# jbikker/tinybvh

Hardware: NVIDIA H100
Metric: Mrays/s (primary+shadow) (higher is better)
Workload: dtype f32

## Files before the change

### tinybvh_b200/csrc/api.cu

```cuda
#include "common.cuh"
#include <stdarg.h>
#include <stdlib.h>
#include <string.h>
#include <vector>
#include <thread>
#include <atomic>
#include <mutex>
#include <condition_variable>
#include <memory>
#include <functional>
#include <new>

static thread_local char g_err[512] = "";
unsigned long long g_tbvh_launches = 0;

void tbvh_set_error( const char* fmt, ... )
{
	va_list ap;
	va_start( ap, fmt );
	vsnprintf( g_err, sizeof( g_err ), fmt, ap );
	va_end( ap );
}

#define ARG_CHECK( c, msg ) do { if (!(c)) { tbvh_set_error( "%s: %s", __func__, msg ); return TBVH_E_ARG; } } while (0)
// ... 670 lines not shown
	ARG_CHECK( instance && blas, "NULL argument" );
	if (!(blas->info.layouts & (1u << TBVH_LAYOUT_BVH))) { tbvh_set_error( "tbvh_instance_update: the BLAS holds no tree" ); return TBVH_E_STATE; }
	return tbvh_instance_update_box( instance, blas->info.aabb_min, blas->info.aabb_max );
}

int tbvh_build_tlas( tbvh_bvh t, const void* instances, uint32_t inst_stride, uint32_t inst_count, const tbvh_bvh* blasses, uint32_t blas_count, float c_trav, float c_int )
{
	ARG_CHECK( t && instances && blasses && inst_count > 0 && blas_count > 0 && inst_stride >= 160, "bad TLAS arguments" );
	CUDA_TRY( cudaSetDevice( t->ctx->device ) );
	free_layouts( t );
	std::vector<float4> boxes( (size_t)inst_count * 2 );
	std::vector<TlasInst> inst( inst_count );
	std::vector<BlasRef> refs( blas_count );
	uint32_t blas_layouts = (1u << TBVH_LAYOUT_BVH) | (1u << TBVH_LAYOUT_CWBVH);
	for (uint32_t k = 0; k < blas_count; k++)
	{
		const tbvh_bvh b = blasses[k];
		ARG_CHECK( b && b != t && b->ctx == t->ctx, "TLAS: a BLAS handle is NULL or lives in another context" );
		const bool has_bvh = (b->info.layouts & (1u << TBVH_LAYOUT_BVH)) && b->d_trav && b->d_leaf_tris, has_cw = b->d_cw_trav && b->d_cw_tris;
		if (b->d_inst || (!has_bvh && !has_cw))
		{ tbvh_set_error( "TLAS: BLAS %u holds no triangle tree (IntersectTLAS walks LAYOUT_BVH BLASses, tiny_bvh.h:3341; traverse_tlas.cl CWBVH ones)", k ); return TBVH_E_STATE; }
		if (has_bvh && b->info.max_depth + 1 > TBVH_STACK) { tbvh_set_error( "TLAS: BLAS %u has depth %u, the two-level kernel walks a BLAS with a %d-entry stack", k, b->info.max_depth, TBVH_STACK ); return TBVH_E_LIMIT; }
		if (has_cw && b->cw_depth + 1 > 128) { tbvh_set_error( "TLAS: the wide tree of BLAS %u has depth %u (128 pending node groups per ray, tiny_bvh.h:7048)", k, b->cw_depth ); return TBVH_E_LIMIT; }
		refs[k].trav = has_bvh ? b->d_trav : 0, refs[k].tris = has_bvh ? b->d_leaf_tris : 0, refs[k].root_ref = b->root_ref, refs[k].root_count = b->root_count, refs[k].pad0 = refs[k].pad1 = 0;
		refs[k].cw_nodes = has_cw ? b->d_cw_trav : 0, refs[k].cw_tris = has_cw ? b->d_cw_tris : 0;
		blas_layouts &= (has_bvh ? 1u << TBVH_LAYOUT_BVH : 0u) | (has_cw ? 1u << TBVH_LAYOUT_CWBVH : 0u);
	}
	for (uint32_t i = 0; i < inst_count; i++)
	{
		const char* r = (const char*)instances + (size_t)i * inst_stride;
		memcpy( inst[i].inv, r + 64, 64 );
		memcpy( &inst[i].blasIdx, r + 140, 4 ), memcpy( &inst[i].mask, r + 156, 4 );
		inst[i].pad0 = inst[i].pad1 = 0;
		ARG_CHECK( inst[i].blasIdx < blas_count, "TLAS: an instance names a BLAS past blas_count" );
		float mn[3], mx[3];
		memcpy( mn, r + 128, 12 ), memcpy( mx, r + 144, 12 );
		boxes[(size_t)i * 2] = make_float4( mn[0], mn[1], mn[2], 0 ), boxes[(size_t)i * 2 + 1] = make_float4( mx[0], mx[1], mx[2], 0 );
	}
	cudaStream_t s = t->ctx->stream;
	CUDA_TRY( cudaMalloc( &t->d_aabbs, boxes.size() * 16 ) );
	CUDA_TRY( cudaMalloc( &t->d_inst, inst.size() * sizeof( TlasInst ) ) );
	CUDA_TRY( cudaMalloc( &t->d_blas, refs.size() * sizeof( BlasRef ) ) );
	CUDA_TRY( cudaMemcpyAsync( t->d_aabbs, boxes.data(), boxes.size() * 16, cudaMemcpyHostToDevice, s ) );
	CUDA_TRY( cudaMemcpyAsync( t->d_inst, inst.data(), inst.size() * sizeof( TlasInst ), cudaMemcpyHostToDevice, s ) );
	CUDA_TRY( cudaMemcpyAsync( t->d_blas, refs.data(), refs.size() * sizeof( BlasRef ), cudaMemcpyHostToDevice, s ) );
	CUDA_TRY( cudaStreamSynchronize( s ) );
	t->info.prim_count = inst_count, t->inst_count = inst_count, t->blas_count = blas_count, t->tlas_blas_layouts = blas_layouts;
	TRY( build_sah_launch( t, c_trav, c_int, TBVH_BUILD_REFERENCE ) );
// ... 390 lines not shown
```

### tinybvh_b200/csrc/common.cuh

```cuda
#pragma once
#include <cuda_runtime.h>
#include <stdint.h>
#include <stdio.h>
#include <mutex>
#include <vector>
#include <atomic>
#include "../../include/tinybvh_b200.h"

#define BVH_FAR 1e30f
#define TBVH_STACK 64
#define TBVH_STACK_DEEP 256

void tbvh_set_error( const char* fmt, ... );
extern unsigned long long g_tbvh_launches;
#define CUDA_TRY( x ) do { cudaError_t e_ = (x); if (e_ != cudaSuccess) { tbvh_set_error( "%s:%d %s -> %s", __FILE__, __LINE__, #x, cudaGetErrorString( e_ ) ); return TBVH_E_CUDA; } } while (0)
#define LAUNCHED() do { g_tbvh_launches++; cudaError_t e_ = cudaGetLastError(); if (e_ != cudaSuccess) { tbvh_set_error( "%s:%d launch -> %s", __FILE__, __LINE__, cudaGetErrorString( e_ ) ); return TBVH_E_CUDA; } } while (0)

struct HostSlot
{
	void* d_rays = 0;
	void* d_hits = 0;
	void* d_bits = 0;
	void* h_hits = 0;
	cudaEvent_t in_done = 0, run_done = 0, out_done = 0;
// ... 32 lines not shown
	std::atomic<uint32_t> counter_next{ 0 };
};
#define TBVH_COUNTERS 256

uint32_t tbvh_next_generation();
struct BlasLink { tbvh_bvh blas; uint32_t generation; };

struct tbvh_bvh_t
{
	tbvh_ctx ctx = 0;
	tbvh_info info = {};
	float4* d_verts = 0;
	float4* d_nodes = 0;
	uint32_t* d_prim_idx = 0;
	float4* d_trav = 0;
	uint32_t root_ref = 0, root_count = 0;
	float4* d_leaf_tris = 0;
	uint32_t leaf_tris_count = 0;
	float4* d_nodes_gpu = 0;
	float4* d_cw_nodes = 0;
	float4* d_cw_tris = 0;
	float4* d_cw_trav = 0;
	uint32_t cw_depth = 0;
	uint32_t generation = 0;
	float4* d_aabbs = 0;
	void* d_inst = 0;
	void* d_blas = 0;
	uint32_t inst_count = 0, blas_count = 0;
	uint32_t tlas_blas_layouts = 0;
	std::vector<BlasLink> links;
	bool refittable = true;
	int stats = 0;
	unsigned long long* d_stats = 0;
};


__device__ __forceinline__ bool mt_test( const float ox, const float oy, const float oz, const float dx, const float dy, const float dz,
	const float4 v0, const float4 e1, const float4 e2, const float tmax, float& t, float& u, float& v )
{
	const float hx = __fmaf_rn( dy, e2.z, -__fmul_rn( dz, e2.y ) );
	const float hy = __fmaf_rn( dz, e2.x, -__fmul_rn( dx, e2.z ) );
	const float hz = __fmaf_rn( dx, e2.y, -__fmul_rn( dy, e2.x ) );
	const float a = __fmaf_rn( e1.z, hz, __fmaf_rn( e1.x, hx, __fmul_rn( e1.y, hy ) ) );
	if (fabsf( a ) < 0.000001f) return false;
	const float f = __fdiv_rn( 1.0f, a );
	const float sx = __fsub_rn( ox, v0.x ), sy = __fsub_rn( oy, v0.y ), sz = __fsub_rn( oz, v0.z );
	u = __fmul_rn( f, __fmaf_rn( hz, sz, __fmaf_rn( hx, sx, __fmul_rn( hy, sy ) ) ) );
	const float qx = __fmaf_rn( -e1.y, sz, __fmul_rn( e1.z, sy ) );
	const float qy = __fmaf_rn( -e1.z, sx, __fmul_rn( e1.x, sz ) );
	const float qz = __fmaf_rn( -e1.x, sy, __fmul_rn( e1.y, sx ) );
	v = __fmul_rn( f, __fmaf_rn( dz, qz, __fmaf_rn( dy, qy, __fmul_rn( dx, qx ) ) ) );
	if (u < 0 || v < 0 || __fadd_rn( u, v ) > 1) return false;
	t = __fmul_rn( f, __fmaf_rn( e2.z, qz, __fmaf_rn( e2.x, qx, __fmul_rn( e2.y, qy ) ) ) );
	return !(t < 0 || t > tmax);
}

__device__ __forceinline__ uint32_t f2key( float f ) { uint32_t u = __float_as_uint( f ); return (u & 0x80000000u) ? ~u : (u | 0x80000000u); }
__device__ __forceinline__ float key2f( uint32_t k ) { return __uint_as_float( (k & 0x80000000u) ? (k & 0x7fffffffu) : ~k ); }

int bvh2_trace_launch( tbvh_bvh b, const void* d_rays, uint32_t stride, void* d_hits, uint32_t hit_stride, uint32_t* d_bits, uint64_t n, bool anyhit, cudaStream_t s, unsigned long long* d_stats );
int cwbvh_trace_launch( tbvh_bvh b, const void* d_rays, uint32_t stride, void* d_hits, uint32_t hit_stride, uint32_t* d_bits, uint64_t n, bool anyhit, cudaStream_t s, unsigned long long* d_stats );
int cw_make_trav( tbvh_bvh b, cudaStream_t s, int known_depth = -1 );
unsigned long long* ctx_next_counter( tbvh_ctx c );
int build_sah_launch( tbvh_bvh b, float c_trav, float c_int, int flavour );
int build_hq_launch( tbvh_bvh b, float c_trav, float c_int );
int refit_launch( tbvh_bvh b, cudaStream_t s );
int tlas_trace_launch( tbvh_bvh b, int layout, const void* d_rays, uint32_t stride, uint32_t* d_bits, uint64_t n, bool anyhit, cudaStream_t s );
struct TlasInst { float inv[16]; uint32_t blasIdx, mask, pad0, pad1; };
struct BlasRef { const float4* trav; const float4* tris; uint32_t root_ref, root_count, pad0, pad1; const float4* cw_nodes; const float4* cw_tris; };
int make_leaf_tris( tbvh_bvh b, cudaStream_t s );
int bvh_gpu_to_bvh( tbvh_bvh b, uint32_t used_nodes_gpu, cudaStream_t s );
int bvh_to_bvh_gpu( tbvh_bvh b, cudaStream_t s );
int bvh_to_cwbvh( tbvh_bvh b, cudaStream_t s );
int exclusive_scan( const uint32_t* in, uint32_t* out, uint32_t* tile_sum, uint32_t n, cudaStream_t s );
```

### tinybvh_b200/csrc/cw_walk.cuh

```cuda
#pragma once
#include "common.cuh"
#include <cuda_fp16.h>

#define CW_STACK 128
#define CW_NODE_F4 10
#ifndef CW_PLANES_BF16
#define CW_PLANES_BF16 0
#endif

__device__ __forceinline__ float2 widen( const uint32_t h2 )
{
#if CW_PLANES_BF16
	return make_float2( __uint_as_float( h2 * 65536u ), __uint_as_float( h2 & 0xffff0000u ) );
#else
	return __half22float2( *(const __half2*)&h2 );
#endif
}

__device__ __forceinline__ float2 fma2( const float2 a, const float2 b, const float2 c )
{
	return make_float2( __fmaf_rn( a.x, b.x, c.x ), __fmaf_rn( a.y, b.y, c.y ) );
}

__device__ __forceinline__ uint32_t pair_hits( const uint32_t wnx, const uint32_t wny, const uint32_t wnz, const uint32_t wfx, const uint32_t wfy, const uint32_t wfz,
	const uint32_t bits_a, const uint32_t bits_b, const float2 ax, const float2 ay, const float2 az, const float2 bx, const float2 by, const float2 bz, const float t )
{
	const float2 tnx = fma2( widen( wnx ), ax, bx ), tny = fma2( widen( wny ), ay, by ), tnz = fma2( widen( wnz ), az, bz );
	const float2 tfx = fma2( widen( wfx ), ax, bx ), tfy = fma2( widen( wfy ), ay, by ), tfz = fma2( widen( wfz ), az, bz );
	const float in_a = fmaxf( fmaxf( fmaxf( tnx.x, tny.x ), tnz.x ), 0.0f ), out_a = fminf( fminf( fminf( tfx.x, tfy.x ), tfz.x ), t );
	const float in_b = fmaxf( fmaxf( fmaxf( tnx.y, tny.y ), tnz.y ), 0.0f ), out_b = fminf( fminf( fminf( tfx.y, tfy.y ), tfz.y ), t );
	return (in_a <= out_a ? bits_a : 0u) | (in_b <= out_b ? bits_b : 0u);
}

__device__ __forceinline__ uint32_t slots_to_order( const uint32_t w, const uint32_t o )
{
	uint32_t top = w >> 24;
	if (o & 1u) top = ((top & 0x55u) << 1) | ((top >> 1) & 0x55u);
	if (o & 2u) top = ((top & 0x33u) << 2) | ((top >> 2) & 0x33u);
	if (o & 4u) top = ((top & 0x0fu) << 4) | (top >> 4);
	return top << 24;
}

template <int OCT> __device__ __forceinline__ uint32_t node_hits( const float4* __restrict__ np, const uint32_t pairs, const bool negx, const bool negy, const bool negz, const uint32_t o,
	const float ax1, const float ay1, const float az1, const float bx1, const float by1, const float bz1, const float t )
{
	const bool nx = OCT < 0 ? negx : (OCT & 4) != 0, ny = OCT < 0 ? negy : (OCT & 2) != 0, nz = OCT < 0 ? negz : (OCT & 1) != 0;
	const float2 ax = make_float2( ax1, ax1 ), ay = make_float2( ay1, ay1 ), az = make_float2( az1, az1 );
	const float2 bx = make_float2( bx1, bx1 ), by = make_float2( by1, by1 ), bz = make_float2( bz1, bz1 );
	(void)pairs;
	float4 A[4], B[4];
	#pragma unroll
	for (int j = 0; j < 4; j++) A[j] = __ldg( np + 2 + 2 * j ), B[j] = __ldg( np + 3 + 2 * j );
	uint32_t got = 0;
	#pragma unroll
	for (int j = 0; j < 4; j++)
	{
		const uint32_t lx = __float_as_uint( A[j].x ), ly = __float_as_uint( A[j].y ), lz = __float_as_uint( A[j].z );
		const uint32_t hx = __float_as_uint( A[j].w ), hy = __float_as_uint( B[j].x ), hz = __float_as_uint( B[j].y );
		got |= pair_hits( nx ? hx : lx, ny ? hy : ly, nz ? hz : lz, nx ? lx : hx, ny ? ly : hy, nz ? lz : hz,
			__float_as_uint( B[j].z ), __float_as_uint( B[j].w ), ax, ay, az, bx, by, bz, t );
	}
	return slots_to_order( got, OCT < 0 ? o : (uint32_t)(7 - OCT) ) | (got & 0x00ffffffu);
}
```

### tinybvh_b200/csrc/multi.cu

```cuda
#include "common.cuh"
#include <sched.h>
#include <sys/mman.h>
#include <string.h>
#include <thread>
#include <string>
#include <vector>
#include <new>

struct tbvh_group_t
{
	std::vector<tbvh_ctx> ctx;
	std::vector<tbvh_bvh> replica;
	std::vector<char> owned;
	std::vector<std::pair<void*, size_t>> host_blocks;
};

#define ARG_CHECK( c, msg ) do { if (!(c)) { tbvh_set_error( "%s: %s", __func__, msg ); return TBVH_E_ARG; } } while (0)
#define TRY( x ) do { int r_ = (x); if (r_ != TBVH_OK) return r_; } while (0)

static void release_replicas( tbvh_group g )
{
	for (size_t i = 0; i < g->replica.size(); i++) if (g->replica[i] && g->owned[i]) tbvh_bvh_destroy( g->replica[i] );
	g->replica.clear(), g->owned.clear();
}
// ... 83 lines not shown
	if (src->d_inst) { tbvh_set_error( "tbvh_group_replicate: a TLAS points into its BLAS handles and cannot be replicated by itself" ); return TBVH_E_UNSUPPORTED; }
	if (!(src->info.layouts & (1u << TBVH_LAYOUT_BVH)) && !src->d_cw_trav) { tbvh_set_error( "tbvh_group_replicate: the source holds no tree" ); return TBVH_E_STATE; }
	release_replicas( g );
	const int sdev = src->ctx->device;
	CUDA_TRY( cudaSetDevice( sdev ) );
	CUDA_TRY( cudaStreamSynchronize( src->ctx->stream ) );
	cudaEvent_t e0 = 0, e1 = 0;
	CUDA_TRY( cudaEventCreate( &e0 ) );
	CUDA_TRY( cudaEventCreate( &e1 ) );
	CUDA_TRY( cudaEventRecord( e0, src->ctx->stream ) );
	int rc = TBVH_OK;
	for (size_t i = 0; i < g->ctx.size() && rc == TBVH_OK; i++)
	{
		tbvh_ctx c = g->ctx[i];
		if (c == src->ctx) { g->replica.push_back( src ), g->owned.push_back( 0 ); continue; }
		tbvh_bvh r = 0;
		rc = tbvh_bvh_create( c, &r );
		if (rc != TBVH_OK) break;
		g->replica.push_back( r ), g->owned.push_back( 1 );
		auto body = [&]() -> int
		{
			CUDA_TRY( cudaSetDevice( c->device ) );
			cudaStream_t s = c->stream;
			r->info = src->info, r->root_ref = src->root_ref, r->root_count = src->root_count, r->refittable = src->refittable, r->cw_depth = src->cw_depth;
			const size_t nodes_b = (size_t)(src->info.used_nodes < 2 ? 2 : src->info.used_nodes) * 32;
			TRY( peer_clone( (void**)&r->d_verts, c->device, src->d_verts, sdev, (size_t)src->info.prim_count * 48, s ) );
			TRY( peer_clone( (void**)&r->d_prim_idx, c->device, src->d_prim_idx, sdev, (size_t)src->info.idx_count * 4, s ) );
			if (src->d_nodes) TRY( peer_clone( (void**)&r->d_nodes, c->device, src->d_nodes, sdev, nodes_b, s ) );
			if (src->d_trav == src->d_nodes) r->d_trav = r->d_nodes;
			else if (src->d_trav) TRY( peer_clone( (void**)&r->d_trav, c->device, src->d_trav, sdev, (size_t)src->info.used_nodes_gpu * 64, s ) );
			if (src->d_leaf_tris) { TRY( peer_clone( (void**)&r->d_leaf_tris, c->device, src->d_leaf_tris, sdev, (size_t)src->leaf_tris_count * 48, s ) ); r->leaf_tris_count = src->leaf_tris_count; }
			if (src->d_nodes_gpu) TRY( peer_clone( (void**)&r->d_nodes_gpu, c->device, src->d_nodes_gpu, sdev, (size_t)src->info.used_nodes_gpu * 64, s ) );
			if (src->d_cw_nodes) TRY( peer_clone( (void**)&r->d_cw_nodes, c->device, src->d_cw_nodes, sdev, (size_t)src->info.used_blocks * 16, s ) );
			if (src->d_cw_tris) TRY( peer_clone( (void**)&r->d_cw_tris, c->device, src->d_cw_tris, sdev, (size_t)src->info.cwbvh_tri_count * 48, s ) );
			if (src->d_cw_trav) TRY( peer_clone( (void**)&r->d_cw_trav, c->device, src->d_cw_trav, sdev, (size_t)(src->info.used_blocks / 5) * 160, s ) );
			return TBVH_OK;
		};
		rc = body();
	}
	for (tbvh_ctx c : g->ctx) { cudaSetDevice( c->device ); cudaStreamSynchronize( c->stream ); }
	cudaSetDevice( sdev );
	cudaEventRecord( e1, src->ctx->stream );
	cudaEventSynchronize( e1 );
	float ms = 0;
	cudaEventElapsedTime( &ms, e0, e1 );
	if (ms_out) *ms_out = ms;
	cudaEventDestroy( e0 ), cudaEventDestroy( e1 );
// ... 71 lines not shown
```

### tinybvh_b200/csrc/trace_cwbvh.cu

```cuda
#include "cw_walk.cuh"
#include <vector>

__global__ void k_cw_expand( const uint4* __restrict__ src, uint4* __restrict__ dst, uint32_t* __restrict__ parent, const uint32_t count )
{
	const uint32_t x = blockIdx.x * blockDim.x + threadIdx.x;
	if (x >= count) return;
	const uint4 n0 = src[(size_t)x * 5], n1 = src[(size_t)x * 5 + 1], n2 = src[(size_t)x * 5 + 2], n3 = src[(size_t)x * 5 + 3], n4 = src[(size_t)x * 5 + 4];
	const uint32_t row[6][2] = { { n2.x, n2.y }, { n2.z, n2.w }, { n3.x, n3.y }, { n3.z, n3.w }, { n4.x, n4.y }, { n4.z, n4.w } };
	const uint32_t meta[2] = { n1.z, n1.w };
	uint32_t word[4][8];
	#pragma unroll
	for (int j = 0; j < 4; j++) for (int k = 0; k < 8; k++) word[j][k] = 0;
	uint32_t kept = 0, inner = 0;
	#pragma unroll
	for (int i = 0; i < 8; i++)
	{
		const uint32_t m = (meta[i >> 2] >> (8 * (i & 3))) & 255u;
		if (m == 0) continue;
		const bool is_inner = (m & 0x18u) == 0x18u;
		const uint32_t bits = is_inner ? 1u << (24u + (m & 7u)) : (m >> 5) << (m & 31u);
		if (is_inner) inner++;
		const uint32_t j = kept >> 1, side = kept & 1;
		#pragma unroll
		for (int r = 0; r < 6; r++)
		{
			const uint32_t q = (row[r][i >> 2] >> (8 * (i & 3))) & 255u;
			const uint32_t h = CW_PLANES_BF16 ? __float_as_uint( (float)q ) >> 16 : (uint32_t)__half_as_ushort( __uint2half_rn( q ) );
			#pragma unroll
			for (int jj = 0; jj < 4; jj++) if (jj == (int)j) word[jj][r] |= side ? h << 16 : h;
		}
// ... 10 lines not shown
	for (int j = 0; j < 4; j++)
	{
		o[2 + 2 * j] = make_uint4( word[j][0], word[j][1], word[j][2], word[j][3] );
		o[3 + 2 * j] = make_uint4( word[j][4], word[j][5], word[j][6], word[j][7] );
	}
	if (parent) for (uint32_t c = 0; c < inner; c++) if (n1.x + c < count) parent[n1.x + c] = x;
}

__global__ void k_cw_depth( const uint32_t* __restrict__ parent, const uint32_t count, uint32_t* __restrict__ max_depth )
{
	const uint32_t x = blockIdx.x * blockDim.x + threadIdx.x;
	if (x >= count) return;
	uint32_t d = 0, n = x;
	while (n != 0 && n < count && d < 4096) n = parent[n], d++;
	if (n != 0) return;
	atomicMax( max_depth, d );
}

int cw_make_trav( tbvh_bvh b, cudaStream_t s, int known_depth )
{
	if (b->d_cw_trav) cudaFree( b->d_cw_trav ), b->d_cw_trav = 0;
	const uint32_t count = b->info.used_blocks / 5;
	if (count == 0) { tbvh_set_error( "cw_make_trav: no CWBVH nodes" ); return TBVH_E_STATE; }
	CUDA_TRY( cudaMalloc( &b->d_cw_trav, (size_t)count * CW_NODE_F4 * 16 ) );
	if (known_depth >= 0)
	{
		k_cw_expand<<<(count + 127) / 128, 128, 0, s>>>( (const uint4*)b->d_cw_nodes, (uint4*)b->d_cw_trav, 0, count ); LAUNCHED();
		b->cw_depth = (uint32_t)known_depth;
		return TBVH_OK;
	}
	uint32_t* d_parent = 0;
	CUDA_TRY( cudaMalloc( &d_parent, ((size_t)count + 1) * 4 ) );
	uint32_t depth = 0;
	auto body = [&]() -> int
	{
		CUDA_TRY( cudaMemsetAsync( d_parent, 0xff, (size_t)count * 4, s ) );
		CUDA_TRY( cudaMemsetAsync( d_parent + count, 0, 4, s ) );
		k_cw_expand<<<(count + 127) / 128, 128, 0, s>>>( (const uint4*)b->d_cw_nodes, (uint4*)b->d_cw_trav, d_parent, count ); LAUNCHED();
		k_cw_depth<<<(count + 127) / 128, 128, 0, s>>>( d_parent, count, d_parent + count ); LAUNCHED();
		CUDA_TRY( cudaMemcpyAsync( &depth, d_parent + count, 4, cudaMemcpyDeviceToHost, s ) );
		CUDA_TRY( cudaStreamSynchronize( s ) );
		return TBVH_OK;
	};
	const int rc = body();
	cudaFree( d_parent );
	b->cw_depth = depth;
	return rc;
}


template <bool ANYHIT, bool STATS, int OCTSW>
__global__ void __launch_bounds__( 128 ) k_trace_wide( const float4* __restrict__ nodes, const float4* __restrict__ tris,
	const char* rays, const uint32_t stride, char* hits, const uint32_t hit_stride, uint32_t* __restrict__ bits, const uint64_t n,
	unsigned long long* __restrict__ stats )
{
	const uint64_t i = (uint64_t)blockIdx.x * blockDim.x + threadIdx.x;
	bool occluded = false;
	const bool valid = i < n;
	float4 ro4 = make_float4( 0, 0, 0, 0 ), rd4 = ro4, rr4 = ro4, rh4 = ro4;
	if (valid)
	{
		const float4* rp = (const float4*)(rays + i * stride);
		ro4 = rp[0], rd4 = rp[1], rr4 = rp[2], rh4 = rp[3];
	}
	const float ox = ro4.x, oy = ro4.y, oz = ro4.z, dx = rd4.x, dy = rd4.y, dz = rd4.z;
	const float rdx = rr4.x, rdy = rr4.y, rdz = rr4.z;
	const uint32_t o = 7u - ((dx < 0 ? 4u : 0u) | (dy < 0 ? 2u : 0u) | (dz < 0 ? 1u : 0u));
	const bool negx = rdx < 0, negy = rdy < 0, negz = rdz < 0;
	const uint32_t oct = (negx ? 4u : 0u) | (negy ? 2u : 0u) | (negz ? 1u : 0u);
	bool uni = false;
	if (OCTSW)
	{
		const uint32_t vm = __ballot_sync( 0xffffffffu, valid );
		const uint32_t oct0 = __shfl_sync( 0xffffffffu, oct, vm ? __ffs( vm ) - 1 : 0 );
		uni = __all_sync( 0xffffffffu, !valid || (oct == oct0 && o == 7u - oct) );
	}
	if (valid)
	{
		float t = rh4.x, hu = rh4.y, hv = rh4.z;
		uint32_t hprim = __float_as_uint( rh4.w );
		uint2 pending[CW_STACK];
		int depth = 0;
		uint32_t base = 0, word = 0x80000000u;
		unsigned long long nsteps = 0, ntris = 0, npairs = 0;
		while (true)
		{
			const uint32_t bit = 31u - __clz( word );
			const uint32_t rest = word & ~(1u << bit);
			if (rest > 0x00ffffffu) pending[depth++] = make_uint2( base, rest );
			const uint32_t slot = (bit - 24u) ^ o;
			const uint32_t nidx = base + __popc( word & ~(0xffffffffu << slot) );
			const float4* np = nodes + (size_t)nidx * CW_NODE_F4;
			const float4 h0 = __ldg( np ), h1 = __ldg( np + 1 );
			if (STATS) nsteps++;
			const uint32_t sxy = __float_as_uint( h0.w ), szm = __float_as_uint( h1.z );
			const float scx = __uint_as_float( sxy << 16 ), scy = __uint_as_float( sxy & 0xffff0000u ), scz = __uint_as_float( szm << 16 );
			const float ax1 = __fmul_rn( scx, rdx ), ay1 = __fmul_rn( scy, rdy ), az1 = __fmul_rn( scz, rdz );
			const float bx1 = __fmul_rn( -__fsub_rn( ox, h0.x ), rdx ), by1 = __fmul_rn( -__fsub_rn( oy, h0.y ), rdy ), bz1 = __fmul_rn( -__fsub_rn( oz, h0.z ), rdz );
			const uint32_t pairs = szm >> 24;
			if (STATS) npairs += pairs;
			uint32_t got;
			#define NODE_HITS( O ) got = node_hits<O>( np, pairs, negx, negy, negz, o, ax1, ay1, az1, bx1, by1, bz1, t )
			if (OCTSW && uni)
			{
				switch (oct)
				{
				case 0: NODE_HITS( 0 ); break;
				case 1: NODE_HITS( 1 ); break;
				case 2: NODE_HITS( 2 ); break;
				case 3: NODE_HITS( 3 ); break;
				case 4: NODE_HITS( 4 ); break;
				case 5: NODE_HITS( 5 ); break;
				case 6: NODE_HITS( 6 ); break;
				default: NODE_HITS( 7 ); break;
				}
			}
			else NODE_HITS( -1 );
			#undef NODE_HITS
			base = __float_as_uint( h1.x );
			word = (got & 0xff000000u) | ((szm >> 16) & 255u);
			uint32_t tmask = got & 0x00ffffffu;
			const float4* tbase = tris + __float_as_uint( h1.y );
			while (tmask)
			{
				const uint32_t k = 31u - __clz( tmask );
				tmask &= ~(1u << k);
				const float4* tp = tbase + k * 3;
				const float4 e2 = __ldg( tp ), e1 = __ldg( tp + 1 ), v0 = __ldg( tp + 2 );
				if (STATS) ntris++;
				float tt, u, v;
				if (mt_test( ox, oy, oz, dx, dy, dz, v0, e1, e2, t, tt, u, v ))
				{
					if (ANYHIT) { occluded = true; break; }
					t = tt, hu = u, hv = v, hprim = __float_as_uint( v0.w );
				}
			}
			if (ANYHIT && occluded) break;
			if (word > 0x00ffffffu) continue;
			if (depth == 0) break;
			const uint2 e = pending[--depth];
			base = e.x, word = e.y;
		}
		if (!ANYHIT)
		{
			float4* hp = (float4*)(hits + i * hit_stride);
			*hp = make_float4( t, hu, hv, __uint_as_float( hprim ) );
		}
		if (STATS) { atomicAdd( &stats[0], nsteps ); atomicAdd( &stats[1], ntris ); atomicAdd( &stats[2], npairs ); }
	}
	if (ANYHIT)
	{
		const uint32_t m = __ballot_sync( 0xffffffffu, occluded );
		if ((threadIdx.x & 31) == 0 && (i & ~31ull) < n) bits[i >> 5] = m;
	}
}

int cwbvh_trace_launch( tbvh_bvh b, const void* d_rays, uint32_t stride, void* d_hits, uint32_t hit_stride, uint32_t* d_bits,
	uint64_t n, bool anyhit, cudaStream_t s, unsigned long long* d_stats )
{
	if (!b->d_cw_trav || !b->d_cw_tris) { tbvh_set_error( "CWBVH layout not resident" ); return TBVH_E_STATE; }
	if (n == 0) return TBVH_OK;
	if (b->cw_depth + 1 > CW_STACK) { tbvh_set_error( "wide-tree depth %u exceeds the %d pending node groups a ray can hold (the reference's own limit)", b->cw_depth, CW_STACK ); return TBVH_E_LIMIT; }
	const uint32_t block = 128;
	const uint64_t grid = (n + block - 1) / block;
	if (grid > 0x7fffffffull) { tbvh_set_error( "ray batch too large for one launch" ); return TBVH_E_ARG; }
	const int sw = b->ctx->trace_variant == 0 ? 0 : 1;
	#define LAUNCH( A, S, O ) k_trace_wide<A, S, O><<<(uint32_t)grid, block, 0, s>>>( b->d_cw_trav, b->d_cw_tris, (const char*)d_rays, stride, \
		(char*)d_hits, hit_stride, d_bits, n, d_stats )
	if (anyhit) { if (d_stats) LAUNCH( true, true, 0 ); else if (sw) LAUNCH( true, false, 1 ); else LAUNCH( true, false, 0 ); }
	else { if (d_stats) LAUNCH( false, true, 0 ); else if (sw) LAUNCH( false, false, 1 ); else LAUNCH( false, false, 0 ); }
	#undef LAUNCH
	LAUNCHED();
	return TBVH_OK;
}
```

### tinybvh_b200/csrc/trace_tlas.cu

```cuda
#include "cw_walk.cuh"

#define TLAS_STACK 64

namespace
{
__device__ __forceinline__ float safercp( const float x ) { return (x > 1e-12f || x < -1e-12f) ? __fdiv_rn( 1.0f, x ) : (x >= 0 ? BVH_FAR : -BVH_FAR); }

__device__ __forceinline__ bool slab( const float4 c0, const float4 c1, const bool px, const bool py, const bool pz, const float rdx, const float rdy, const float rdz,
	const float nrox, const float nroy, const float nroz, const float tmax, float& tmin )
{
	const float tx1 = __fmaf_rn( px ? c0.x : c1.x, rdx, nrox ), tx2 = __fmaf_rn( px ? c1.x : c0.x, rdx, nrox );
	const float ty1 = __fmaf_rn( py ? c0.y : c1.y, rdy, nroy ), ty2 = __fmaf_rn( py ? c1.y : c0.y, rdy, nroy );
	const float tz1 = __fmaf_rn( pz ? c0.z : c1.z, rdz, nroz ), tz2 = __fmaf_rn( pz ? c1.z : c0.z, rdz, nroz );
	tmin = fmaxf( fmaxf( tx1, ty1 ), fmaxf( tz1, 0.0f ) );
	return fminf( fminf( tx2, ty2 ), fminf( tz2, tmax ) ) >= tmin;
}

template <bool ANYHIT> __device__ bool trace_blas( const BlasRef B, const float ox, const float oy, const float oz, const float dx, const float dy, const float dz,
	const float rdx, const float rdy, const float rdz, float& tmax, float& hu, float& hv, uint32_t& hprim, bool& hit, uint2* stack )
{
	const bool px = dx >= 0, py = dy >= 0, pz = dz >= 0;
	const float nrox = -__fmul_rn( ox, rdx ), nroy = -__fmul_rn( oy, rdy ), nroz = -__fmul_rn( oz, rdz );
	int sp = 0;
	uint32_t ref = B.root_ref, cnt = B.root_count;
// ... 18 lines not shown
			if (hitb) { ref = refb, cnt = cntb; continue; }
		}
		else
		{
			const float4* tp = B.tris + (size_t)ref * 3;
			for (uint32_t k = 0; k < cnt; k++, tp += 3)
			{
				const float4 v0 = __ldg( tp ), e1 = __ldg( tp + 1 ), e2 = __ldg( tp + 2 );
				float t, u, v;
				if (mt_test( ox, oy, oz, dx, dy, dz, v0, e1, e2, tmax, t, u, v ))
				{
					if (ANYHIT) return true;
					tmax = t, hu = u, hv = v, hprim = __float_as_uint( v0.w ), hit = true;
				}
			}
		}
		if (sp == 0) break;
		const uint2 e = stack[--sp];
		ref = e.x, cnt = e.y;
	}
	return false;
}

template <bool ANYHIT> __device__ bool trace_blas_cw( const float4* __restrict__ nodes, const float4* __restrict__ tris, const float ox, const float oy, const float oz,
	const float dx, const float dy, const float dz, const float rdx, const float rdy, const float rdz, float& tmax, float& hu, float& hv, uint32_t& hprim, bool& hit, uint2* pending )
{
	const uint32_t o = 7u - ((dx < 0 ? 4u : 0u) | (dy < 0 ? 2u : 0u) | (dz < 0 ? 1u : 0u));
	const bool negx = rdx < 0, negy = rdy < 0, negz = rdz < 0;
	const float t_in = tmax;
	float t = tmax, lu = 0, lv = 0;
	uint32_t lprim = 0;
	int depth = 0;
	uint32_t base = 0, word = 0x80000000u;
	while (true)
	{
		const uint32_t bit = 31u - __clz( word );
		const uint32_t rest = word & ~(1u << bit);
		if (rest > 0x00ffffffu) pending[depth++] = make_uint2( base, rest );
		const uint32_t slot = (bit - 24u) ^ o;
		const uint32_t nidx = base + __popc( word & ~(0xffffffffu << slot) );
		const float4* np = nodes + (size_t)nidx * CW_NODE_F4;
		const float4 h0 = __ldg( np ), h1 = __ldg( np + 1 );
		const uint32_t sxy = __float_as_uint( h0.w ), szm = __float_as_uint( h1.z );
		const float scx = __uint_as_float( sxy << 16 ), scy = __uint_as_float( sxy & 0xffff0000u ), scz = __uint_as_float( szm << 16 );
		const float ax1 = __fmul_rn( scx, rdx ), ay1 = __fmul_rn( scy, rdy ), az1 = __fmul_rn( scz, rdz );
		const float bx1 = __fmul_rn( -__fsub_rn( ox, h0.x ), rdx ), by1 = __fmul_rn( -__fsub_rn( oy, h0.y ), rdy ), bz1 = __fmul_rn( -__fsub_rn( oz, h0.z ), rdz );
		const uint32_t got = node_hits<-1>( np, szm >> 24, negx, negy, negz, o, ax1, ay1, az1, bx1, by1, bz1, t );
		base = __float_as_uint( h1.x );
		word = (got & 0xff000000u) | ((szm >> 16) & 255u);
		uint32_t tmask = got & 0x00ffffffu;
		const float4* tbase = tris + __float_as_uint( h1.y );
		while (tmask)
		{
			const uint32_t k = 31u - __clz( tmask );
			tmask &= ~(1u << k);
			const float4* tp = tbase + k * 3;
			const float4 e2 = __ldg( tp ), e1 = __ldg( tp + 1 ), v0 = __ldg( tp + 2 );
			float tt, u, v;
			if (mt_test( ox, oy, oz, dx, dy, dz, v0, e1, e2, t, tt, u, v ))
			{
				if (ANYHIT) { if (tt < t_in) return true; }
				else t = tt, lu = u, lv = v, lprim = __float_as_uint( v0.w );
			}
		}
		if (word > 0x00ffffffu) continue;
		if (depth == 0) break;
		const uint2 e = pending[--depth];
		base = e.x, word = e.y;
	}
	if (!ANYHIT && t < t_in) tmax = t, hu = lu, hv = lv, hprim = lprim, hit = true;
// ... 37 lines not shown
					continue;
				}
				if (hita) { ref = refa, cnt = cnta; continue; }
				if (hitb) { ref = refb, cnt = cntb; continue; }
			}
			else
			{
				for (uint32_t k = 0; k < cnt; k++)
				{
					const uint32_t instIdx = __ldg( prim_idx + ref + k );
					const float4* ip = (const float4*)(inst + instIdx);
					const float4 r0 = __ldg( ip ), r1 = __ldg( ip + 1 ), r2 = __ldg( ip + 2 ), r3 = __ldg( ip + 3 ), meta = __ldg( ip + 4 );
					if (!(__float_as_uint( meta.y ) & rmask)) continue;
					float tox = __fadd_rn( __fmaf_rn( r0.z, oz, __fmaf_rn( r0.x, ox, __fmul_rn( r0.y, oy ) ) ), r0.w );
					float toy = __fadd_rn( __fmaf_rn( r1.z, oz, __fmaf_rn( r1.x, ox, __fmul_rn( r1.y, oy ) ) ), r1.w );
					float toz = __fadd_rn( __fmaf_rn( r2.z, oz, __fmaf_rn( r2.x, ox, __fmul_rn( r2.y, oy ) ) ), r2.w );
					const float w = __fadd_rn( __fmaf_rn( oz, r3.z, __fmaf_rn( ox, r3.x, __fmul_rn( oy, r3.y ) ) ), r3.w );
					if (!(w == 1.0f)) { const float rw = __fdiv_rn( 1.0f, w ); tox = __fmul_rn( tox, rw ), toy = __fmul_rn( toy, rw ), toz = __fmul_rn( toz, rw ); }
					const float tdx = __fmaf_rn( r0.z, dz, __fmaf_rn( r0.x, dx, __fmul_rn( r0.y, dy ) ) );
					const float tdy = __fmaf_rn( r1.z, dz, __fmaf_rn( r1.x, dx, __fmul_rn( r1.y, dy ) ) );
					const float tdz = __fmaf_rn( r2.z, dz, __fmaf_rn( r2.x, dx, __fmul_rn( r2.y, dy ) ) );
					bool hit = false;
					const BlasRef B = blas[__float_as_uint( meta.x )];
					const bool occ = CW ? trace_blas_cw<ANYHIT>( B.cw_nodes, B.cw_tris, tox, toy, toz, tdx, tdy, tdz, safercp( tdx ), safercp( tdy ), safercp( tdz ), tmax, hu, hv, hprim, hit, bstack )
						: trace_blas<ANYHIT>( B, tox, toy, toz, tdx, tdy, tdz, safercp( tdx ), safercp( tdy ), safercp( tdz ), tmax, hu, hv, hprim, hit, bstack );
					if (occ)
					{
						occluded = true;
						break;
					}
					if (hit)
					{
						hinst = instIdx;
						if (inst_shift) hprim += instIdx << inst_shift;
					}
				}
				if (ANYHIT && occluded) break;
			}
			if (sp == 0) break;
			const uint2 e = stack[--sp];
			ref = e.x, cnt = e.y;
		}
		if (!ANYHIT)
		{
			char* rec = rays + i * stride;
			if (inst_shift == 0) *(uint32_t*)(rec + 44) = hinst;
			*(float4*)(rec + 48) = make_float4( tmax, hu, hv, __uint_as_float( hprim ) );
		}
// ... 32 lines not shown
```

Baseline: 2788.

## Use integer min/max slab test for CWBVH nodes when ray ranges fit

Computes a per-BLAS exponent bound on node scales during wide-tree expansion and derives a reciprocal-direction limit. When every ray in a warp fits that bound, the node slab test uses integer vimax3/vimin3 comparisons on float bit patterns instead of chains of fmaxf/fminf. It also hoists the per-octant specialization out to the whole traversal loop rather than switching per node. The cost is more template instantiations, larger code, and an extra atomic reduction plus readback during tree preparation.

```diff
diff --git a/tinybvh_b200/csrc/api.cu b/tinybvh_b200/csrc/api.cu
--- a/tinybvh_b200/csrc/api.cu
+++ b/tinybvh_b200/csrc/api.cu
@@ -716,8 +716,8 @@
 		{ tbvh_set_error( "TLAS: BLAS %u holds no triangle tree (IntersectTLAS walks LAYOUT_BVH BLASses, tiny_bvh.h:3341; traverse_tlas.cl CWBVH ones)", k ); return TBVH_E_STATE; }
 		if (has_bvh && b->info.max_depth + 1 > TBVH_STACK) { tbvh_set_error( "TLAS: BLAS %u has depth %u, the two-level kernel walks a BLAS with a %d-entry stack", k, b->info.max_depth, TBVH_STACK ); return TBVH_E_LIMIT; }
 		if (has_cw && b->cw_depth + 1 > 128) { tbvh_set_error( "TLAS: the wide tree of BLAS %u has depth %u (128 pending node groups per ray, tiny_bvh.h:7048)", k, b->cw_depth ); return TBVH_E_LIMIT; }
-		refs[k].trav = has_bvh ? b->d_trav : 0, refs[k].tris = has_bvh ? b->d_leaf_tris : 0, refs[k].root_ref = b->root_ref, refs[k].root_count = b->root_count, refs[k].pad0 = refs[k].pad1 = 0;
-		refs[k].cw_nodes = has_cw ? b->d_cw_trav : 0, refs[k].cw_tris = has_cw ? b->d_cw_tris : 0;
+		refs[k].trav = has_bvh ? b->d_trav : 0, refs[k].tris = has_bvh ? b->d_leaf_tris : 0, refs[k].root_ref = b->root_ref, refs[k].root_count = b->root_count, refs[k].pad1 = 0;
+		refs[k].cw_nodes = has_cw ? b->d_cw_trav : 0, refs[k].cw_tris = has_cw ? b->d_cw_tris : 0, refs[k].cw_rd_limit = has_cw ? b->cw_rd_limit : -1.0f;
 		blas_layouts &= (has_bvh ? 1u << TBVH_LAYOUT_BVH : 0u) | (has_cw ? 1u << TBVH_LAYOUT_CWBVH : 0u);
 	}
 	for (uint32_t i = 0; i < inst_count; i++)
diff --git a/tinybvh_b200/csrc/common.cuh b/tinybvh_b200/csrc/common.cuh
--- a/tinybvh_b200/csrc/common.cuh
+++ b/tinybvh_b200/csrc/common.cuh
@@ -78,6 +78,7 @@
 	float4* d_cw_tris = 0;
 	float4* d_cw_trav = 0;
 	uint32_t cw_depth = 0;
+	float cw_rd_limit = -1.0f;
 	uint32_t generation = 0;
 	float4* d_aabbs = 0;
 	void* d_inst = 0;
@@ -123,7 +124,7 @@
 int refit_launch( tbvh_bvh b, cudaStream_t s );
 int tlas_trace_launch( tbvh_bvh b, int layout, const void* d_rays, uint32_t stride, uint32_t* d_bits, uint64_t n, bool anyhit, cudaStream_t s );
 struct TlasInst { float inv[16]; uint32_t blasIdx, mask, pad0, pad1; };
-struct BlasRef { const float4* trav; const float4* tris; uint32_t root_ref, root_count, pad0, pad1; const float4* cw_nodes; const float4* cw_tris; };
+struct BlasRef { const float4* trav; const float4* tris; uint32_t root_ref, root_count; float cw_rd_limit; uint32_t pad1; const float4* cw_nodes; const float4* cw_tris; };
 int make_leaf_tris( tbvh_bvh b, cudaStream_t s );
 int bvh_gpu_to_bvh( tbvh_bvh b, uint32_t used_nodes_gpu, cudaStream_t s );
 int bvh_to_bvh_gpu( tbvh_bvh b, cudaStream_t s );
diff --git a/tinybvh_b200/csrc/cw_walk.cuh b/tinybvh_b200/csrc/cw_walk.cuh
--- a/tinybvh_b200/csrc/cw_walk.cuh
+++ b/tinybvh_b200/csrc/cw_walk.cuh
@@ -22,11 +22,19 @@
 	return make_float2( __fmaf_rn( a.x, b.x, c.x ), __fmaf_rn( a.y, b.y, c.y ) );
 }
 
-__device__ __forceinline__ uint32_t pair_hits( const uint32_t wnx, const uint32_t wny, const uint32_t wnz, const uint32_t wfx, const uint32_t wfy, const uint32_t wfz,
+template <bool IORD> __device__ __forceinline__ uint32_t pair_hits( const uint32_t wnx, const uint32_t wny, const uint32_t wnz, const uint32_t wfx, const uint32_t wfy, const uint32_t wfz,
 	const uint32_t bits_a, const uint32_t bits_b, const float2 ax, const float2 ay, const float2 az, const float2 bx, const float2 by, const float2 bz, const float t )
 {
 	const float2 tnx = fma2( widen( wnx ), ax, bx ), tny = fma2( widen( wny ), ay, by ), tnz = fma2( widen( wnz ), az, bz );
 	const float2 tfx = fma2( widen( wfx ), ax, bx ), tfy = fma2( widen( wfy ), ay, by ), tfz = fma2( widen( wfz ), az, bz );
+	if (IORD)
+	{
+		const int in_a = __vimax3_s32_relu( __float_as_int( tnx.x ), __float_as_int( tny.x ), __float_as_int( tnz.x ) );
+		const int in_b = __vimax3_s32_relu( __float_as_int( tnx.y ), __float_as_int( tny.y ), __float_as_int( tnz.y ) );
+		const int out_a = __vimin3_s32( __float_as_int( tfx.x ), __float_as_int( tfy.x ), __float_as_int( tfz.x ) );
+		const int out_b = __vimin3_s32( __float_as_int( tfx.y ), __float_as_int( tfy.y ), __float_as_int( tfz.y ) );
+		return (in_a <= out_a && !(__int_as_float( in_a ) > t) ? bits_a : 0u) | (in_b <= out_b && !(__int_as_float( in_b ) > t) ? bits_b : 0u);
+	}
 	const float in_a = fmaxf( fmaxf( fmaxf( tnx.x, tny.x ), tnz.x ), 0.0f ), out_a = fminf( fminf( fminf( tfx.x, tfy.x ), tfz.x ), t );
 	const float in_b = fmaxf( fmaxf( fmaxf( tnx.y, tny.y ), tnz.y ), 0.0f ), out_b = fminf( fminf( fminf( tfx.y, tfy.y ), tfz.y ), t );
 	return (in_a <= out_a ? bits_a : 0u) | (in_b <= out_b ? bits_b : 0u);
@@ -41,13 +49,24 @@
 	return top << 24;
 }
 
-template <int OCT> __device__ __forceinline__ uint32_t node_hits( const float4* __restrict__ np, const uint32_t pairs, const bool negx, const bool negy, const bool negz, const uint32_t o,
-	const float ax1, const float ay1, const float az1, const float bx1, const float by1, const float bz1, const float t )
+#define CW_ORIGIN_LIMIT 8.5070592e37f
+__device__ __forceinline__ bool cw_ray_fits( const float ox, const float oy, const float oz, const float rdx, const float rdy, const float rdz, const float rd_limit )
 {
+	return fabsf( rdx ) <= rd_limit && fabsf( rdy ) <= rd_limit && fabsf( rdz ) <= rd_limit &&
+		fabsf( ox ) <= CW_ORIGIN_LIMIT && fabsf( oy ) <= CW_ORIGIN_LIMIT && fabsf( oz ) <= CW_ORIGIN_LIMIT;
+}
+
+template <int OCT, bool IORD> __device__ __forceinline__ uint32_t node_hits( const float4* __restrict__ np, const float4 h0, const float4 h1,
+	const float ox, const float oy, const float oz, const float rdx, const float rdy, const float rdz, const bool negx, const bool negy, const bool negz, const uint32_t o, const float t )
+{
+	const uint32_t sxy = __float_as_uint( h0.w ), szm = __float_as_uint( h1.z );
+	const float scx = __uint_as_float( sxy << 16 ), scy = __uint_as_float( sxy & 0xffff0000u ), scz = __uint_as_float( szm << 16 );
+	const float ax1 = __fmul_rn( scx, rdx ), ay1 = __fmul_rn( scy, rdy ), az1 = __fmul_rn( scz, rdz );
+	const float bx1 = __fadd_rn( __fmul_rn( -__fsub_rn( ox, h0.x ), rdx ), 0.0f ), by1 = __fadd_rn( __fmul_rn( -__fsub_rn( oy, h0.y ), rdy ), 0.0f );
+	const float bz1 = __fadd_rn( __fmul_rn( -__fsub_rn( oz, h0.z ), rdz ), 0.0f );
 	const bool nx = OCT < 0 ? negx : (OCT & 4) != 0, ny = OCT < 0 ? negy : (OCT & 2) != 0, nz = OCT < 0 ? negz : (OCT & 1) != 0;
 	const float2 ax = make_float2( ax1, ax1 ), ay = make_float2( ay1, ay1 ), az = make_float2( az1, az1 );
 	const float2 bx = make_float2( bx1, bx1 ), by = make_float2( by1, by1 ), bz = make_float2( bz1, bz1 );
-	(void)pairs;
 	float4 A[4], B[4];
 	#pragma unroll
 	for (int j = 0; j < 4; j++) A[j] = __ldg( np + 2 + 2 * j ), B[j] = __ldg( np + 3 + 2 * j );
@@ -57,7 +76,7 @@
 	{
 		const uint32_t lx = __float_as_uint( A[j].x ), ly = __float_as_uint( A[j].y ), lz = __float_as_uint( A[j].z );
 		const uint32_t hx = __float_as_uint( A[j].w ), hy = __float_as_uint( B[j].x ), hz = __float_as_uint( B[j].y );
-		got |= pair_hits( nx ? hx : lx, ny ? hy : ly, nz ? hz : lz, nx ? lx : hx, ny ? ly : hy, nz ? lz : hz,
+		got |= pair_hits<IORD>( nx ? hx : lx, ny ? hy : ly, nz ? hz : lz, nx ? lx : hx, ny ? ly : hy, nz ? lz : hz,
 			__float_as_uint( B[j].z ), __float_as_uint( B[j].w ), ax, ay, az, bx, by, bz, t );
 	}
 	return slots_to_order( got, OCT < 0 ? o : (uint32_t)(7 - OCT) ) | (got & 0x00ffffffu);
diff --git a/tinybvh_b200/csrc/multi.cu b/tinybvh_b200/csrc/multi.cu
--- a/tinybvh_b200/csrc/multi.cu
+++ b/tinybvh_b200/csrc/multi.cu
@@ -129,7 +129,7 @@
 		{
 			CUDA_TRY( cudaSetDevice( c->device ) );
 			cudaStream_t s = c->stream;
-			r->info = src->info, r->root_ref = src->root_ref, r->root_count = src->root_count, r->refittable = src->refittable, r->cw_depth = src->cw_depth;
+			r->info = src->info, r->root_ref = src->root_ref, r->root_count = src->root_count, r->refittable = src->refittable, r->cw_depth = src->cw_depth, r->cw_rd_limit = src->cw_rd_limit;
 			const size_t nodes_b = (size_t)(src->info.used_nodes < 2 ? 2 : src->info.used_nodes) * 32;
 			TRY( peer_clone( (void**)&r->d_verts, c->device, src->d_verts, sdev, (size_t)src->info.prim_count * 48, s ) );
 			TRY( peer_clone( (void**)&r->d_prim_idx, c->device, src->d_prim_idx, sdev, (size_t)src->info.idx_count * 4, s ) );
diff --git a/tinybvh_b200/csrc/trace_cwbvh.cu b/tinybvh_b200/csrc/trace_cwbvh.cu
--- a/tinybvh_b200/csrc/trace_cwbvh.cu
+++ b/tinybvh_b200/csrc/trace_cwbvh.cu
@@ -1,11 +1,19 @@
 #include "cw_walk.cuh"
 #include <vector>
 
-__global__ void k_cw_expand( const uint4* __restrict__ src, uint4* __restrict__ dst, uint32_t* __restrict__ parent, const uint32_t count )
+__global__ void k_cw_expand( const uint4* __restrict__ src, uint4* __restrict__ dst, uint32_t* __restrict__ parent, uint32_t* __restrict__ range, const uint32_t count )
 {
 	const uint32_t x = blockIdx.x * blockDim.x + threadIdx.x;
 	if (x >= count) return;
 	const uint4 n0 = src[(size_t)x * 5], n1 = src[(size_t)x * 5 + 1], n2 = src[(size_t)x * 5 + 2], n3 = src[(size_t)x * 5 + 3], n4 = src[(size_t)x * 5 + 4];
+	{
+		const int ex = (int8_t)(n0.w & 255u), ey = (int8_t)((n0.w >> 8) & 255u), ez = (int8_t)((n0.w >> 16) & 255u);
+		const bool p_ok = fabsf( __uint_as_float( n0.x ) ) <= CW_ORIGIN_LIMIT && fabsf( __uint_as_float( n0.y ) ) <= CW_ORIGIN_LIMIT && fabsf( __uint_as_float( n0.z ) ) <= CW_ORIGIN_LIMIT;
+		const bool bad = !p_ok || ex == -128 || ey == -128 || ez == -128;
+		const uint32_t key = bad ? 256u : (uint32_t)(128 + max( ex, max( ey, ez ) ));
+		const uint32_t m = __reduce_max_sync( __activemask(), key );
+		if ((threadIdx.x & 31) == __ffs( __activemask() ) - 1) atomicMax( range, m );
+	}
 	const uint32_t row[6][2] = { { n2.x, n2.y }, { n2.z, n2.w }, { n3.x, n3.y }, { n3.z, n3.w }, { n4.x, n4.y }, { n4.z, n4.w } };
 	const uint32_t meta[2] = { n1.z, n1.w };
 	uint32_t word[4][8];
@@ -62,37 +70,90 @@
 	if (b->d_cw_trav) cudaFree( b->d_cw_trav ), b->d_cw_trav = 0;
 	const uint32_t count = b->info.used_blocks / 5;
 	if (count == 0) { tbvh_set_error( "cw_make_trav: no CWBVH nodes" ); return TBVH_E_STATE; }
-	CUDA_TRY( cudaMalloc( &b->d_cw_trav, (size_t)count * CW_NODE_F4 * 16 ) );
-	if (known_depth >= 0)
-	{
-		k_cw_expand<<<(count + 127) / 128, 128, 0, s>>>( (const uint4*)b->d_cw_nodes, (uint4*)b->d_cw_trav, 0, count ); LAUNCHED();
-		b->cw_depth = (uint32_t)known_depth;
-		return TBVH_OK;
-	}
+	CUDA_TRY( cudaMalloc( &b->d_cw_trav, ((size_t)count * CW_NODE_F4 + 1) * 16 ) );
+	uint32_t* d_range = (uint32_t*)(b->d_cw_trav + (size_t)count * CW_NODE_F4);
+	uint32_t range = 256;
+	b->cw_rd_limit = -1.0f;
+	CUDA_TRY( cudaMemsetAsync( d_range, 0, 4, s ) );
 	uint32_t* d_parent = 0;
-	CUDA_TRY( cudaMalloc( &d_parent, ((size_t)count + 1) * 4 ) );
-	uint32_t depth = 0;
+	uint32_t depth = (uint32_t)known_depth;
 	auto body = [&]() -> int
 	{
-		CUDA_TRY( cudaMemsetAsync( d_parent, 0xff, (size_t)count * 4, s ) );
-		CUDA_TRY( cudaMemsetAsync( d_parent + count, 0, 4, s ) );
-		k_cw_expand<<<(count + 127) / 128, 128, 0, s>>>( (const uint4*)b->d_cw_nodes, (uint4*)b->d_cw_trav, d_parent, count ); LAUNCHED();
-		k_cw_depth<<<(count + 127) / 128, 128, 0, s>>>( d_parent, count, d_parent + count ); LAUNCHED();
-		CUDA_TRY( cudaMemcpyAsync( &depth, d_parent + count, 4, cudaMemcpyDeviceToHost, s ) );
+		if (known_depth >= 0) k_cw_expand<<<(count + 127) / 128, 128, 0, s>>>( (const uint4*)b->d_cw_nodes, (uint4*)b->d_cw_trav, 0, d_range, count );
+		else
+		{
+			CUDA_TRY( cudaMalloc( &d_parent, ((size_t)count + 1) * 4 ) );
+			CUDA_TRY( cudaMemsetAsync( d_parent, 0xff, (size_t)count * 4, s ) );
+			CUDA_TRY( cudaMemsetAsync( d_parent + count, 0, 4, s ) );
+			k_cw_expand<<<(count + 127) / 128, 128, 0, s>>>( (const uint4*)b->d_cw_nodes, (uint4*)b->d_cw_trav, d_parent, d_range, count ); LAUNCHED();
+			k_cw_depth<<<(count + 127) / 128, 128, 0, s>>>( d_parent, count, d_parent + count );
+			CUDA_TRY( cudaMemcpyAsync( &depth, d_parent + count, 4, cudaMemcpyDeviceToHost, s ) );
+		}
+		LAUNCHED();
+		CUDA_TRY( cudaMemcpyAsync( &range, d_range, 4, cudaMemcpyDeviceToHost, s ) );
 		CUDA_TRY( cudaStreamSynchronize( s ) );
 		return TBVH_OK;
 	};
 	const int rc = body();
-	cudaFree( d_parent );
+	if (d_parent) cudaFree( d_parent );
 	b->cw_depth = depth;
+	if (rc == TBVH_OK && range < 256) b->cw_rd_limit = ldexpf( 1.0f, 127 - max( 0, (int)range - 128 ) );
 	return rc;
 }
 
+
+template <bool ANYHIT, bool STATS, int OCT, bool IORD> __device__ __forceinline__ bool cw_trace( const float4* __restrict__ nodes, const float4* __restrict__ tris,
+	const float ox, const float oy, const float oz, const float dx, const float dy, const float dz, const float rdx, const float rdy, const float rdz,
+	const uint32_t o, const bool negx, const bool negy, const bool negz, float& t, float& hu, float& hv, uint32_t& hprim, uint2* pending, unsigned long long* __restrict__ stats )
+{
+	int depth = 0;
+	uint32_t base = 0, word = 0x80000000u;
+	unsigned long long nsteps = 0, ntris = 0, npairs = 0;
+	bool occluded = false;
+	while (true)
+	{
+		const uint32_t bit = 31u - __clz( word );
+		const uint32_t rest = word & ~(1u << bit);
+		if (rest > 0x00ffffffu) pending[depth++] = make_uint2( base, rest );
+		const uint32_t slot = (bit - 24u) ^ (OCT < 0 ? o : (uint32_t)(7 - OCT));
+		const uint32_t nidx = base + __popc( word & ~(0xffffffffu << slot) );
+		const float4* np = nodes + (size_t)nidx * CW_NODE_F4;
+		const float4 h0 = __ldg( np ), h1 = __ldg( np + 1 );
+		const uint32_t szm = __float_as_uint( h1.z );
+		if (STATS) nsteps++, npairs += szm >> 24;
+		const uint32_t got = node_hits<OCT, IORD>( np, h0, h1, ox, oy, oz, rdx, rdy, rdz, negx, negy, negz, o, t );
+		base = __float_as_uint( h1.x );
+		word = (got & 0xff000000u) | ((szm >> 16) & 255u);
+		uint32_t tmask = got & 0x00ffffffu;
+		const float4* tbase = tris + __float_as_uint( h1.y );
+		while (tmask)
+		{
+			const uint32_t k = 31u - __clz( tmask );
+			tmask &= ~(1u << k);
+			const float4* tp = tbase + k * 3;
+			const float4 e2 = __ldg( tp ), e1 = __ldg( tp + 1 ), v0 = __ldg( tp + 2 );
+			if (STATS) ntris++;
+			float tt, u, v;
+			if (mt_test( ox, oy, oz, dx, dy, dz, v0, e1, e2, t, tt, u, v ))
+			{
+				if (ANYHIT) { occluded = true; break; }
+				t = tt, hu = u, hv = v, hprim = __float_as_uint( v0.w );
+			}
+		}
+		if (ANYHIT && occluded) break;
+		if (word > 0x00ffffffu) continue;
+		if (depth == 0) break;
+		const uint2 e = pending[--depth];
+		base = e.x, word = e.y;
+	}
+	if (STATS) { atomicAdd( &stats[0], nsteps ); atomicAdd( &stats[1], ntris ); atomicAdd( &stats[2], npairs ); }
+	return occluded;
+}
 
 template <bool ANYHIT, bool STATS, int OCTSW>
 __global__ void __launch_bounds__( 128 ) k_trace_wide( const float4* __restrict__ nodes, const float4* __restrict__ tris,
 	const char* rays, const uint32_t stride, char* hits, const uint32_t hit_stride, uint32_t* __restrict__ bits, const uint64_t n,
-	unsigned long long* __restrict__ stats )
+	unsigned long long* __restrict__ stats, const float rd_limit )
 {
 	const uint64_t i = (uint64_t)blockIdx.x * blockDim.x + threadIdx.x;
 	bool occluded = false;
@@ -115,78 +176,35 @@
 		const uint32_t oct0 = __shfl_sync( 0xffffffffu, oct, vm ? __ffs( vm ) - 1 : 0 );
 		uni = __all_sync( 0xffffffffu, !valid || (oct == oct0 && o == 7u - oct) );
 	}
+	const bool iord = __all_sync( 0xffffffffu, !valid || cw_ray_fits( ox, oy, oz, rdx, rdy, rdz, rd_limit ) );
 	if (valid)
 	{
 		float t = rh4.x, hu = rh4.y, hv = rh4.z;
 		uint32_t hprim = __float_as_uint( rh4.w );
 		uint2 pending[CW_STACK];
-		int depth = 0;
-		uint32_t base = 0, word = 0x80000000u;
-		unsigned long long nsteps = 0, ntris = 0, npairs = 0;
-		while (true)
-		{
-			const uint32_t bit = 31u - __clz( word );
-			const uint32_t rest = word & ~(1u << bit);
-			if (rest > 0x00ffffffu) pending[depth++] = make_uint2( base, rest );
-			const uint32_t slot = (bit - 24u) ^ o;
-			const uint32_t nidx = base + __popc( word & ~(0xffffffffu << slot) );
-			const float4* np = nodes + (size_t)nidx * CW_NODE_F4;
-			const float4 h0 = __ldg( np ), h1 = __ldg( np + 1 );
-			if (STATS) nsteps++;
-			const uint32_t sxy = __float_as_uint( h0.w ), szm = __float_as_uint( h1.z );
-			const float scx = __uint_as_float( sxy << 16 ), scy = __uint_as_float( sxy & 0xffff0000u ), scz = __uint_as_float( szm << 16 );
-			const float ax1 = __fmul_rn( scx, rdx ), ay1 = __fmul_rn( scy, rdy ), az1 = __fmul_rn( scz, rdz );
-			const float bx1 = __fmul_rn( -__fsub_rn( ox, h0.x ), rdx ), by1 = __fmul_rn( -__fsub_rn( oy, h0.y ), rdy ), bz1 = __fmul_rn( -__fsub_rn( oz, h0.z ), rdz );
-			const uint32_t pairs = szm >> 24;
-			if (STATS) npairs += pairs;
-			uint32_t got;
-			#define NODE_HITS( O ) got = node_hits<O>( np, pairs, negx, negy, negz, o, ax1, ay1, az1, bx1, by1, bz1, t )
-			if (OCTSW && uni)
+		#define TRACE( O, I ) occluded = cw_trace<ANYHIT, STATS, O, I>( nodes, tris, ox, oy, oz, dx, dy, dz, rdx, rdy, rdz, o, negx, negy, negz, t, hu, hv, hprim, pending, stats )
+		if (OCTSW && uni && iord)
+		{
+			switch (oct)
 			{
-				switch (oct)
-				{
-				case 0: NODE_HITS( 0 ); break;
-				case 1: NODE_HITS( 1 ); break;
-				case 2: NODE_HITS( 2 ); break;
-				case 3: NODE_HITS( 3 ); break;
-				case 4: NODE_HITS( 4 ); break;
-				case 5: NODE_HITS( 5 ); break;
-				case 6: NODE_HITS( 6 ); break;
-				default: NODE_HITS( 7 ); break;
-				}
+			case 0: TRACE( 0, true ); break;
+			case 1: TRACE( 1, true ); break;
+			case 2: TRACE( 2, true ); break;
+			case 3: TRACE( 3, true ); break;
+			case 4: TRACE( 4, true ); break;
+			case 5: TRACE( 5, true ); break;
+			case 6: TRACE( 6, true ); break;
+			default: TRACE( 7, true ); break;
 			}
-			else NODE_HITS( -1 );
-			#undef NODE_HITS
-			base = __float_as_uint( h1.x );
-			word = (got & 0xff000000u) | ((szm >> 16) & 255u);
-			uint32_t tmask = got & 0x00ffffffu;
-			const float4* tbase = tris + __float_as_uint( h1.y );
-			while (tmask)
-			{
-				const uint32_t k = 31u - __clz( tmask );
-				tmask &= ~(1u << k);
-				const float4* tp = tbase + k * 3;
-				const float4 e2 = __ldg( tp ), e1 = __ldg( tp + 1 ), v0 = __ldg( tp + 2 );
-				if (STATS) ntris++;
-				float tt, u, v;
-				if (mt_test( ox, oy, oz, dx, dy, dz, v0, e1, e2, t, tt, u, v ))
-				{
-					if (ANYHIT) { occluded = true; break; }
-					t = tt, hu = u, hv = v, hprim = __float_as_uint( v0.w );
-				}
-			}
-			if (ANYHIT && occluded) break;
-			if (word > 0x00ffffffu) continue;
-			if (depth == 0) break;
-			const uint2 e = pending[--depth];
-			base = e.x, word = e.y;
-		}
+		}
+		else if (iord) TRACE( -1, true );
+		else TRACE( -1, false );
+		#undef TRACE
 		if (!ANYHIT)
 		{
 			float4* hp = (float4*)(hits + i * hit_stride);
 			*hp = make_float4( t, hu, hv, __uint_as_float( hprim ) );
 		}
-		if (STATS) { atomicAdd( &stats[0], nsteps ); atomicAdd( &stats[1], ntris ); atomicAdd( &stats[2], npairs ); }
 	}
 	if (ANYHIT)
 	{
@@ -206,7 +224,7 @@
 	if (grid > 0x7fffffffull) { tbvh_set_error( "ray batch too large for one launch" ); return TBVH_E_ARG; }
 	const int sw = b->ctx->trace_variant == 0 ? 0 : 1;
 	#define LAUNCH( A, S, O ) k_trace_wide<A, S, O><<<(uint32_t)grid, block, 0, s>>>( b->d_cw_trav, b->d_cw_tris, (const char*)d_rays, stride, \
-		(char*)d_hits, hit_stride, d_bits, n, d_stats )
+		(char*)d_hits, hit_stride, d_bits, n, d_stats, b->cw_rd_limit )
 	if (anyhit) { if (d_stats) LAUNCH( true, true, 0 ); else if (sw) LAUNCH( true, false, 1 ); else LAUNCH( true, false, 0 ); }
 	else { if (d_stats) LAUNCH( false, true, 0 ); else if (sw) LAUNCH( false, false, 1 ); else LAUNCH( false, false, 0 ); }
 	#undef LAUNCH
diff --git a/tinybvh_b200/csrc/trace_tlas.cu b/tinybvh_b200/csrc/trace_tlas.cu
--- a/tinybvh_b200/csrc/trace_tlas.cu
+++ b/tinybvh_b200/csrc/trace_tlas.cu
@@ -64,7 +64,7 @@
 	return false;
 }
 
-template <bool ANYHIT> __device__ bool trace_blas_cw( const float4* __restrict__ nodes, const float4* __restrict__ tris, const float ox, const float oy, const float oz,
+template <bool ANYHIT, bool IORD> __device__ bool trace_blas_cw( const float4* __restrict__ nodes, const float4* __restrict__ tris, const float ox, const float oy, const float oz,
 	const float dx, const float dy, const float dz, const float rdx, const float rdy, const float rdz, float& tmax, float& hu, float& hv, uint32_t& hprim, bool& hit, uint2* pending )
 {
 	const uint32_t o = 7u - ((dx < 0 ? 4u : 0u) | (dy < 0 ? 2u : 0u) | (dz < 0 ? 1u : 0u));
@@ -83,11 +83,8 @@
 		const uint32_t nidx = base + __popc( word & ~(0xffffffffu << slot) );
 		const float4* np = nodes + (size_t)nidx * CW_NODE_F4;
 		const float4 h0 = __ldg( np ), h1 = __ldg( np + 1 );
-		const uint32_t sxy = __float_as_uint( h0.w ), szm = __float_as_uint( h1.z );
-		const float scx = __uint_as_float( sxy << 16 ), scy = __uint_as_float( sxy & 0xffff0000u ), scz = __uint_as_float( szm << 16 );
-		const float ax1 = __fmul_rn( scx, rdx ), ay1 = __fmul_rn( scy, rdy ), az1 = __fmul_rn( scz, rdz );
-		const float bx1 = __fmul_rn( -__fsub_rn( ox, h0.x ), rdx ), by1 = __fmul_rn( -__fsub_rn( oy, h0.y ), rdy ), bz1 = __fmul_rn( -__fsub_rn( oz, h0.z ), rdz );
-		const uint32_t got = node_hits<-1>( np, szm >> 24, negx, negy, negz, o, ax1, ay1, az1, bx1, by1, bz1, t );
+		const uint32_t szm = __float_as_uint( h1.z );
+		const uint32_t got = node_hits<-1, IORD>( np, h0, h1, ox, oy, oz, rdx, rdy, rdz, negx, negy, negz, o, t );
 		base = __float_as_uint( h1.x );
 		word = (got & 0xff000000u) | ((szm >> 16) & 255u);
 		uint32_t tmask = got & 0x00ffffffu;
@@ -171,8 +168,12 @@
 					const float tdz = __fmaf_rn( r2.z, dz, __fmaf_rn( r2.x, dx, __fmul_rn( r2.y, dy ) ) );
 					bool hit = false;
 					const BlasRef B = blas[__float_as_uint( meta.x )];
-					const bool occ = CW ? trace_blas_cw<ANYHIT>( B.cw_nodes, B.cw_tris, tox, toy, toz, tdx, tdy, tdz, safercp( tdx ), safercp( tdy ), safercp( tdz ), tmax, hu, hv, hprim, hit, bstack )
-						: trace_blas<ANYHIT>( B, tox, toy, toz, tdx, tdy, tdz, safercp( tdx ), safercp( tdy ), safercp( tdz ), tmax, hu, hv, hprim, hit, bstack );
+					const float trdx = safercp( tdx ), trdy = safercp( tdy ), trdz = safercp( tdz );
+					bool occ;
+					if (!CW) occ = trace_blas<ANYHIT>( B, tox, toy, toz, tdx, tdy, tdz, trdx, trdy, trdz, tmax, hu, hv, hprim, hit, bstack );
+					else if (cw_ray_fits( tox, toy, toz, trdx, trdy, trdz, B.cw_rd_limit ))
+						occ = trace_blas_cw<ANYHIT, true>( B.cw_nodes, B.cw_tris, tox, toy, toz, tdx, tdy, tdz, trdx, trdy, trdz, tmax, hu, hv, hprim, hit, bstack );
+					else occ = trace_blas_cw<ANYHIT, false>( B.cw_nodes, B.cw_tris, tox, toy, toz, tdx, tdy, tdz, trdx, trdy, trdz, tmax, hu, hv, hprim, hit, bstack );
 					if (occ)
 					{
 						occluded = true;
```

New measurement: 3318 (median of 6 runs). 1.19x the previous value.
